# qrp73/SDRPP

Hardware: AMD Instinct MI355X
Metric: IQ Msamples/s through FFT+FIR+demod chain; % HBM roofline at 1/2/4/8 GPU (higher is better)
Workload: dtype f32

## Files before the change

sdrpp_amd/csrc/fft.hip:

```cpp
#include <cmath>
#include <cstring>
#include <cstdlib>
#include <algorithm>
#include <utility>
#include "sdrgpu_internal.h"
#include "fft_stages.h"
#include "fir_rows.h"
#include "fir_tail.h"

#ifndef SDRGPU_PB_NT
#define SDRGPU_PB_NT 1
#endif
#ifndef SDRGPU_PA_CP
#define SDRGPU_PA_CP 2
#endif
namespace sdrgpu {

__device__ __forceinline__ float db_of(float2 X) {
    const float p = X.x * X.x + X.y * X.y;
    int e;
    const float m = frexpf(p, &e);
    const double l = (double)e + (double)__builtin_amdgcn_logf(m);
    return (float)(3.0102999566398119521 * l);
}
// ... 631 lines not shown

namespace op1 {
constexpr int M = 16384;
constexpr int RS = 560;
constexpr int TW512 = 32 * RS;
constexpr int W128 = TW512 + 512;
constexpr int W128D = (W128 + 64) * 8;
constexpr int LDS_BYTES = W128D + 64 * 16;
constexpr int TAB = 512 + 128;
constexpr int TAB64 = 2048 + 128;
}

__device__ __forceinline__ float2 wmul(float2 x, float w) {
#pragma clang fp contract(off)
    return make_float2(x.x * w, x.y * w);
}

__device__ __forceinline__ void dft32(float2* v) {
    constexpr float C[16] = {1.0f, 0.98078528040323044913f, 0.92387953251128675613f, 0.83146961230254523708f,
                             0.70710678118654752440f, 0.55557023301960222474f, 0.38268343236508977173f,
                             0.19509032201612826785f, 0.0f, -0.19509032201612826785f, -0.38268343236508977173f,
                             -0.55557023301960222474f, -0.70710678118654752440f, -0.83146961230254523708f,
                             -0.92387953251128675613f, -0.98078528040323044913f};
    float2 e[16], o[16];
#pragma unroll
    for (int i = 0; i < 16; i++) {
        e[i] = v[2 * i];
        o[i] = v[2 * i + 1];
    }
    dft16(e);
    dft16(o);
#pragma unroll
    for (int k = 0; k < 16; k++) {
        float2 t = o[k];
        if (k == 8) t = mul_negi(t);
        else if (k) t = cmul(t, make_float2(C[k], -C[(k + 8) & 15] * (k < 8 ? -1.0f : 1.0f)));
        v[k] = cadd(e[k], t);
        v[k + 16] = csub(e[k], t);
    }
}

constexpr int k1pSlots = 5;
constexpr int k1pPB = 2;
#ifndef SDRGPU_1P_ABL
#define SDRGPU_1P_ABL 0
#endif
#ifndef SDRGPU_1P_EARLYDMA
#define SDRGPU_1P_EARLYDMA 1
#endif
#ifndef SDRGPU_1P_EARLYW128
#define SDRGPU_1P_EARLYW128 1
#endif
#ifdef SDRGPU_1P_TIMING
__device__ unsigned long long g_1p_t[16384 * 8];
#define T1P(k)                                                                                    \
    do {                                                                                          \
        if (threadIdx.x == 0 && blockIdx.x < 16384) g_1p_t[blockIdx.x * 8 + (k)] = clock64();     \
    } while (0)
#else
#define T1P(k) do {} while (0)
#endif
__device__ __forceinline__ void vfo_half_block(const VfoWork& v, int g, int p) {
    const int lane = threadIdx.x & 63, wave = threadIdx.x >> 6;
#pragma unroll 1
    for (int k = 0; k < 2; k++) {
        const long long seg = (long long)(v.frame0 + g) * 64 + p * 32 + k * 16 + wave * 2 + (lane >> 5);
        fir_rows_segment<32, 5, true, false, 32, 32, true>(v.a, seg, lane);
    }
}
template <bool ZM, bool VFO, bool PAD>
__global__ __launch_bounds__(512) __attribute__((amdgpu_waves_per_eu(1))) void fft_1p_kernel(
    const float2* __restrict__ in, long long frameStride, int frames, const float* __restrict__ win, int nz,
    const float2* __restrict__ tab, const double2* __restrict__ tab64, float* __restrict__ out, float* __restrict__ zpart,
    VfoWork v) {
    using op1::M;
    using op1::RS;
    using op1::TW512;
    using op1::W128;
    extern __shared__ __attribute__((aligned(16))) float2 lds[];
    if constexpr (VFO) {
        if (v.hist && blockIdx.x == gridDim.x - 1) {
            (void)fir_hist_block<float2, true, false>(v.a);
            return;
        }
    }
    const int b = blockIdx.x, k = b >> 3;
    const int f = 8 * (k >> 1) + (b & 7), p = k & 1, r0 = 2 * p;
    if (f >= frames) return;
    T1P(0);
    constexpr bool kDma = !PAD && !(SDRGPU_1P_ABL & 1);
    constexpr bool kVfo = VFO && !(SDRGPU_1P_ABL & 4);
    if constexpr (kVfo && !(kDma && SDRGPU_1P_EARLYDMA)) vfo_half_block(v, f, p);
    T1P(1);
    auto tid = [] {
        int u = threadIdx.x;
        asm volatile("" : "+v"(u));
        return u;
    };
    {
        const int t = threadIdx.x;
        lds[TW512 + t] = tab[t];
        if (t < 64) reinterpret_cast<double2*>(reinterpret_cast<char*>(lds) + op1::W128D)[t] = tab64[2048 + 32 * (r0 + (t >> 5)) + (t & 31)];
    }
    const float fxa = p ? -1.0f : 1.0f, fyb = p ? 1.0f : -1.0f;
    auto combine2 = [&](const float2 (&u)[4], float2& ya, float2& yb) {
        const float2 aa = cadd(u[0], u[2]), qa = cadd(u[1], u[3]), ab = csub(u[0], u[2]), qb = csub(u[1], u[3]);
        ya = make_float2(fmaf(fxa, qa.x, aa.x), fmaf(fxa, qa.y, aa.y));
        yb = make_float2(fmaf(-fyb, qb.y, ab.x), fmaf(fyb, qb.x, ab.y));
    };
    const unsigned lim = PAD ? (unsigned)nz : 65536u;
    const __amdgpu_buffer_rsrc_t rw = brsrc(win, lim * 4u);
    const __amdgpu_buffer_rsrc_t rx = brsrc(in + (long long)f * frameStride, lim * 8u);
    constexpr int PB = k1pPB, NB = 32 / PB;
    float2 za[32], zb[32];
    float2 xv[2][PB][4];
    float wv[2][PB][4];
    auto issue = [&](auto bbc) {
        constexpr int bb = decltype(bbc)::value;
        const int t = tid();
#pragma unroll
        for (int ii = 0; ii < PB; ii++)
#pragma unroll
            for (int j = 0; j < 4; j++) {
                const int n0 = 512 * (PB * bb + ii) + M * j;
                if constexpr (PAD) {
                    xv[bb & 1][ii][j] = __builtin_bit_cast(float2, __builtin_amdgcn_raw_buffer_load_b64(rx, (t + n0) * 8, 0, 0));
                    wv[bb & 1][ii][j] = __builtin_bit_cast(float, __builtin_amdgcn_raw_buffer_load_b32(rw, (t + n0) * 4, 0, 0));
                } else {
                    xv[bb & 1][ii][j] = __builtin_bit_cast(float2, __builtin_amdgcn_raw_buffer_load_b64(rx, t * 8, n0 * 8, 0));
                    wv[bb & 1][ii][j] = __builtin_bit_cast(float, __builtin_amdgcn_raw_buffer_load_b32(rw, t * 4, n0 * 4, 0));
                }
            }
    };
    auto step = [&](auto bbc) {
        constexpr int bb = decltype(bbc)::value;
#pragma unroll
        for (int ii = 0; ii < PB; ii++) {
            float2 u[4];
#pragma unroll
            for (int j = 0; j < 4; j++) u[j] = wmul(xv[bb & 1][ii][j], wv[bb & 1][ii][j]);
            combine2(u, za[PB * bb + ii], zb[PB * bb + ii]);

        }
        if constexpr (bb + 2 < NB) issue(std::integral_constant<int, bb + 2>{});
        __builtin_amdgcn_sched_barrier(0);
    };
    if constexpr (SDRGPU_1P_ABL & 1) {
#pragma unroll
        for (int i = 0; i < 32; i++) {
            za[i] = make_float2((float)(tid() + i), (float)i);
            zb[i] = make_float2((float)i, (float)(tid() - i));
        }
    } else if constexpr (PAD) {
        issue(std::integral_constant<int, 0>{});
        issue(std::integral_constant<int, 1>{});
        static_for<0, NB>(step);
    } else {
        constexpr int S = k1pSlots, SLOT = 24576;
        typedef __attribute__((address_space(3))) char lchar;
        const unsigned ldsBase = (unsigned)(size_t)(lchar*)lds;
        const int wave = __builtin_amdgcn_readfirstlane(threadIdx.x >> 6);
        const char* gb[3];
        unsigned rstep[3], loff[3];
        const float2* xf = in + (long long)f * frameStride;
#pragma unroll
        for (int e = 0; e < 3; e++) {
            const int m = 3 * wave + e;
            const int jx = m >> 2, cx = m & 3, jw = (m - 16) >> 1, cw = (m - 16) & 1;
            gb[e] = m < 16 ? reinterpret_cast<const char*>(xf + M * jx + 128 * cx)
                           : reinterpret_cast<const char*>(win + M * jw + 256 * cw);
            rstep[e] = m < 16 ? 512u * 8u : 512u * 4u;
            loff[e] = m < 16 ? (unsigned)(4096 * jx + 1024 * cx) : (unsigned)(16384 + 2048 * jw + 1024 * cw);
        }
        auto dma = [&](auto ic) {
            constexpr int i = decltype(ic)::value;
            const unsigned lane16 = (unsigned)(tid() & 63) * 16u;
#pragma unroll
            for (int e = 0; e < 3; e++) {
                const char* src = gb[e] + lane16;
                gb[e] += rstep[e];
                asm volatile("" : "+s"(gb[e]));
                const unsigned dst = __builtin_amdgcn_readfirstlane(ldsBase + (unsigned)((i % S) * SLOT) + loff[e]);
                unsigned keep;
                asm volatile("s_mov_b32 %0, m0\n\ts_mov_b32 m0, %2\n\ts_nop 0\n\tglobal_load_lds_dwordx4 %1, off\n\ts_mov_b32 m0, %0"
                             : "=&s"(keep) : "v"(src), "s"(dst) : "memory");
            }
        };
        static_for<0, S - 1>(dma);
        if constexpr (kVfo && SDRGPU_1P_EARLYDMA) vfo_half_block(v, f, p);
        static_for<0, 32>([&](auto ic) {
            constexpr int i = decltype(ic)::value;
            constexpr int younger = (S - 2 < 31 - i) ? S - 2 : 31 - i;
            asm volatile("s_waitcnt vmcnt(%0)" ::"n"(3 * younger) : "memory");
            __builtin_amdgcn_s_barrier();
            asm volatile("" ::: "memory");
            if constexpr (i + S - 1 < 32) dma(std::integral_constant<int, i + S - 1>{});
            const int t = tid();
            const char* slot = reinterpret_cast<const char*>(lds) + (i % S) * SLOT;
            float2 u[4];
#pragma unroll
            for (int j = 0; j < 4; j++) {
                const float2 xx = *reinterpret_cast<const float2*>(slot + 4096 * j + 8 * t);
                const float ww = *reinterpret_cast<const float*>(slot + 16384 + 2048 * j + 4 * t);
                u[j] = wmul(xx, ww);
            }
            combine2(u, za[i], zb[i]);
            __builtin_amdgcn_sched_barrier(0);
        });
    }
    T1P(2);
    float* zf = ZM ? zpart + ((long long)f << 12) : nullptr;
    const __amdgpu_buffer_rsrc_t ro = brsrc(out + ((long long)f << 16), 65536u * 4u);
    float dA[2][16];
    constexpr bool kEarlyW = SDRGPU_1P_EARLYW128 && VFO;
    auto w128mul = [&](float2 (&z)[32], int hh) {
        const double2* w128 = reinterpret_cast<const double2*>(reinterpret_cast<const char*>(lds) + op1::W128D) + 32 * hh;
#pragma unroll
        for (int i = 1; i < 32; i++) {
            const double2 q = zmul(make_double2(z[i].x, z[i].y), w128[i]);
            z[i] = make_float2((float)q.x, (float)q.y);
        }
    };
    auto transform = [&](auto hc, float2 (&z)[32]) {
        constexpr int h = decltype(hc)::value;
        const int r = r0 + h;
        __syncthreads();
        {
            const int t = tid();
            if constexpr (!(kEarlyW && h == 1)) w128mul(z, h);
            dft32(z);
            const double2 st = tab64[4 * t];
            double2 ce = tab64[t * r], co = zmul(ce, st);
            const double2 st2 = zmul(st, st);
            float2* row = lds + pad16(t);
            if constexpr (SDRGPU_1P_ABL & 8) {
                const float2 cf = make_float2((float)ce.x, (float)ce.y), sf = make_float2((float)st.x, (float)st.y);
#pragma unroll
                for (int k2 = 0; k2 < 32; k2++) row[k2 * RS] = cmul(z[k2], k2 & 1 ? sf : cf);
            } else
#pragma unroll
            for (int k2 = 0; k2 < 32; k2 += 2) {
                row[k2 * RS] = cmul(z[k2], make_float2((float)ce.x, (float)ce.y));
                row[(k2 + 1) * RS] = cmul(z[k2 + 1], make_float2((float)co.x, (float)co.y));
                if (k2 < 30) {
                    ce = zmul(ce, st2);
                    co = zmul(co, st2);
                }
            }
        }
        __syncthreads();
        if constexpr (h == 0) T1P(5);
        {
            const int t = tid();
            const int k2 = t >> 4, t0 = t & 15;
            float2 a[32];
            const float2* src = lds + k2 * RS + t0;
#pragma unroll
            for (int t1 = 0; t1 < 32; t1++) a[t1] = src[17 * t1];
            dft32(a);
#pragma unroll
            for (int q1 = 1; q1 < 32; q1++) a[q1] = cmul(a[q1], lds[TW512 + 16 * q1 + t0]);
            __syncthreads();
            float2* dst = lds + k2 * RS + (t0 ^ ((k2 >> 1) & 15));
#pragma unroll
            for (int q1 = 0; q1 < 32; q1++) dst[17 * q1] = a[q1];
        }
        __syncthreads();
        T1P(6 + h);
        static_for<0, 2>([&](auto ec) {
            constexpr int e = decltype(ec)::value;
            const int t = tid();
            const int pe = t + 512 * e, k2 = pe & 31, q1 = pe >> 5, sw = (k2 >> 1) & 15;
            float2 c3[16];
            const float2* src = lds + k2 * RS + 17 * q1;
#pragma unroll
            for (int t0 = 0; t0 < 16; t0++) c3[t0] = src[t0 ^ sw];
            if constexpr (kEarlyW && h == 0 && e == 0) w128mul(zb, 1);
            dft16(c3);
            if constexpr (SDRGPU_1P_ABL & 16) {
                if constexpr (h == 1) {
                    float acc = 0.0f;
#pragma unroll
                    for (int q2 = 0; q2 < 16; q2++) acc += c3[q2].x + c3[q2].y;
                    out[(f << 16) + pe] = acc;
                }
            } else if constexpr (h == 0) {
#pragma unroll
                for (int q2 = 0; q2 < 16; q2++) dA[e][q2] = db_of(c3[q2]);
            } else {
                float dv[16];
                const unsigned vo = (unsigned)(4 * (k2 + 32 * q1) + r0) * 4u;
#pragma unroll
                for (int q2 = 0; q2 < 16; q2++) {
                    dv[q2] = db_of(c3[q2]);
                    __builtin_amdgcn_raw_buffer_store_b64(__builtin_bit_cast(bu2, make_float2(dA[e][q2], dv[q2])), ro, vo,
                                                          q2 * 4096 * 4, 0);
                }
                if constexpr (ZM) {
#pragma unroll
                    for (int q2 = 0; q2 < 16; q2++) dv[q2] = fmaxf(dA[e][q2], dv[q2]);
                    const int lane = t & 63;
                    tr_step<1, 8>(dv, lane);
                    tr_step<2, 4>(dv, lane);
                    tr_step<4, 2>(dv, lane);
                    const int q2 = ((lane & 1) << 3) | ((lane & 2) << 1) | (lane & 4) >> 1;
                    float* zp = zf + ((long long)p << 11) + (k2 >> 3) + 4 * q1 + 128 * q2;
                    zp[0] = dv[0];
                    zp[128] = dv[1];
                }
            }
        });
    };
    if constexpr (SDRGPU_1P_ABL & 2) {
        float2 acc = make_float2(0.0f, 0.0f);
#pragma unroll
        for (int i = 0; i < 32; i++) acc = cadd(acc, cadd(za[i], zb[i]));
        out[(f << 16) + tid()] = acc.x + acc.y;
        return;
    }
    transform(std::integral_constant<int, 0>{}, za);
    T1P(3);
    transform(std::integral_constant<int, 1>{}, zb);
    T1P(4);
}

#ifdef SDRGPU_1P_TIMING
extern "C" int sdrgpu_debug_1p_times(unsigned long long* host, int n) {
    return hipMemcpyFromSymbol(host, HIP_SYMBOL(g_1p_t), sizeof(unsigned long long) * (size_t)n) == hipSuccess ? 0 : -1;
}
#endif

static_assert(TAIL_NT_BIG == 256, "zoom_fold_block's indexing and the fold's block count assume 256 threads");
__device__ __forceinline__ void zoom_fold_block(const float* __restrict__ zpart, int frames, float* __restrict__ zoom, int blk) {
    const long long i = ((long long)blk * 256 + threadIdx.x) * 4;
    if (i >= (long long)frames * 2048) return;
    const long long f = i >> 11, o = i & 2047;
    const float4 a = *reinterpret_cast<const float4*>(zpart + (f << 12) + o);
    const float4 b = *reinterpret_cast<const float4*>(zpart + (f << 12) + 2048 + o);
    const float4 m = make_float4(fmaxf(a.x, b.x), fmaxf(a.y, b.y), fmaxf(a.z, b.z), fmaxf(a.w, b.w));
    if (((uintptr_t)zoom & 15) == 0) {
        *reinterpret_cast<float4*>(zoom + i) = m;
    } else {
        zoom[i] = m.x; zoom[i + 1] = m.y; zoom[i + 2] = m.z; zoom[i + 3] = m.w;
    }
}
__global__ __launch_bounds__(256) void fft_1p_zoom_kernel(const float* __restrict__ zpart, int frames, float* __restrict__ zoom) {
    zoom_fold_block(zpart, frames, zoom, blockIdx.x);
}
__global__ __launch_bounds__(TAIL_NT_BIG) void fft_1p_tail_fold_kernel(TailArgs t, const float* __restrict__ zpart, int frames,
                                                                         float* __restrict__ zoom) {
    extern __shared__ __attribute__((aligned(16))) float2 XS[];
    __shared__ TailGeom gs[TAIL_MAXS];
    const int w = blockIdx.x;
    if (w < t.G) fir_tail_block<TAIL_K_BIG, TAIL_NT_BIG>(t, w, w == t.G - 1, XS, gs);
    else zoom_fold_block(zpart, frames, zoom, w - t.G);
}

struct VfoCall {
    FirArgs a;
    int blocks;
};
__global__ __launch_bounds__(512) __attribute__((amdgpu_waves_per_eu(4))) void fft_passA_vfo_kernel(
    const float2* __restrict__ in, long long frameStride, int frames, const float* __restrict__ win, int nz, int N2,
    int logN, const float2* __restrict__ tw, const float2* __restrict__ tfull, float2* __restrict__ scratch,
    const float2* __restrict__ headp, int nh, SideCopy side, VfoCall v) {
    extern __shared__ __attribute__((aligned(16))) float2 lds[];
    const int ntiles = (N2 / 32) * frames;
    int b = blockIdx.x;
    if (b < ntiles) {
        passA_tile<256, 32>(lds, b, in, frameStride, frames, win, nz, N2, logN, tw, tfull, scratch, headp, nh);
        return;
    }
    b -= ntiles;
    if (b < v.blocks) {
        const int lane = threadIdx.x & 63, wave = threadIdx.x >> 6;
        fir_rows_segment<32, 5, true, false, 32, 32, true>(v.a, ((long long)b * 8 + wave) * 2 + (lane >> 5), lane);
        return;
    }
    b -= v.blocks;
    if (b == 0) {
        fir_hist_copy<float2, true, false>(v.a);
        return;
    }
    const int w = b - 1, nw = gridDim.x - ntiles - v.blocks - 1;
    for (int k = 0; k < side.count; k++)
        for (int i = w * blockDim.x + threadIdx.x; i < side.n[k]; i += nw * blockDim.x) side.dst[k][i] = side.src[k][i];
}

__global__ __launch_bounds__(512) __attribute__((amdgpu_waves_per_eu(4))) void fft_passB_tail_kernel(
    const float2* __restrict__ scratch, int frames, int N1, int logN, const float2* __restrict__ tw, float* __restrict__ out,
    TailArgs t) {
    extern __shared__ __attribute__((aligned(16))) float2 lds[];
    __shared__ TailGeom gs[TAIL_MAXS];
    const int ntiles = (N1 / 32) * frames;
    if ((int)blockIdx.x < ntiles) {
        passB_tile<256, 32, false>(lds, blockIdx.x, scratch, frames, N1, logN, tw, out, nullptr);
        return;
    }
    const int w = blockIdx.x - ntiles;
    fir_tail_block<TAIL_K, TAIL_NT>(t, w, w == t.G - 1, lds, gs);
}

struct FftPlan {
    int device = 0, N = 0, logN = 0, nz = 0;
    int N1 = 0, N2 = 0;
    DevBuf win, tw1, tw2, tfull, scratch, scratch2;
    int chunkFrames = 1;
    int sa = 16, sb = 32;
    float2* cur = nullptr;
    int sa2 = 0;
    int gridA = 0, gridB = 0;
    DevBuf wt;
    hipStream_t own = nullptr;
    PinnedBuf pin_in, pin_out;
    DevBuf dev_in, dev_out;
    int merge = 1;
    StreamOrder order;
    sdrgpu_zoom* zoom = nullptr;
    int zoomSize = 0;
    Fft64Plan* f64 = nullptr;
    static constexpr int kTimed = 256;
    bool timing = false;
    hipEvent_t tev[kTimed][2] = {};
    long long tcalls = 0;
    int vfoFuse = 1;
    int onepass = 0;
    DevBuf tab1p, tab1p64, zpart;
    hipStream_t tailStream = nullptr;
    DevBuf s1T[2], zpartT[2];
    hipEvent_t gdone[2] = {}, tdone[2] = {};
    bool tdoneRec[2] = {};
    long long tcallsT = 0;
};
static int time_mark(FftPlan& p, int which, hipStream_t s) {
    if (!p.timing) return SDRGPU_OK;
    SDRGPU_HIP(hipEventRecord(p.tev[p.tcalls % FftPlan::kTimed][which], s));
    if (which == 1) p.tcalls++;
    return SDRGPU_OK;
}

static int make_twiddles(DevBuf& b, int L, int count = -1, int step = 1) {
    if (count < 0) count = L;
    std::vector<float2> t(count);
    for (int m = 0; m < count; m++) {
        double a = -2.0 * M_PI * (double)((long long)m * step % L) / (double)L;
        t[m] = make_float2((float)std::cos(a), (float)std::sin(a));
    }
    SDRGPU_CHECK(b.ensure(sizeof(float2) * count));
    SDRGPU_HIP(hipMemcpy(b.p, t.data(), sizeof(float2) * count, hipMemcpyHostToDevice));
    return SDRGPU_OK;
}

template <typename K>
static int set_lds(K kernel, size_t bytes) {
    SDRGPU_HIP(hipFuncSetAttribute((const void*)kernel, hipFuncAttributeMaxDynamicSharedMemorySize, (int)bytes));
    return SDRGPU_OK;
}

template <int L, int S>
static int launch_single(const FftPlan& p, const float2* in, long long stride, int frames, float* out, hipStream_t s) {
    auto k = fft_single_kernel<L, S>;
    size_t lds = sizeof(float2) * S * Lds<L>::LS;
    SDRGPU_CHECK(set_lds(k, lds));
    dim3 grid((frames + S - 1) / S);
    hipLaunchKernelGGL(k, grid, dim3(S * L / 16), lds, s, in, stride, frames, p.win.as<float>(), p.nz,
                       p.tw1.as<float2>(), out);
    SDRGPU_HIP(hipGetLastError());
    return SDRGPU_OK;
}

template <int L, int S>
static int launch_passA(const FftPlan& p, const float2* in, long long stride, int frames, hipStream_t s,
                        const float2* headp = nullptr, int nh = 0, const SideCopy* side = nullptr) {
    auto k = fft_passA_kernel<L, S>;
    size_t lds = sizeof(float2) * (S * Lds<L>::LS + (L == 256 ? L + 256 : 0));
    SDRGPU_CHECK(set_lds(k, lds));
    SideCopy sc{};
    int spare = 0;
    if (side && side->count > 0) {
// ... 135 lines not shown
    set_error("fft: unsupported N2 %d", p.N2);
    return SDRGPU_EARG;
}

}

using namespace sdrgpu;

struct sdrgpu_fft {
    FftPlan p;
};

static int fft_upload_window(sdrgpu_fft* h, const float* window, int nz) {
    if (nz <= 0 || nz > h->p.N) { set_error("fft: nz %d out of range (N %d)", nz, h->p.N); return SDRGPU_EARG; }
    SDRGPU_SET_DEVICE(h->p.device);
    SDRGPU_CHECK(h->p.win.ensure(sizeof(float) * nz));
    SDRGPU_HIP(hipMemcpy(h->p.win.p, window, sizeof(float) * nz, hipMemcpyHostToDevice));
    h->p.nz = nz;
    return SDRGPU_OK;
}

extern "C" int sdrgpu_fft_create(sdrgpu_fft** out, int device, int fftSize, int nz, int windowType) {
    if (!out) { set_error("fft_create: null handle"); return SDRGPU_EARG; }
    *out = nullptr;
    int logN = 0;
    while ((1 << logN) < fftSize) logN++;
    if (fftSize < 64 || fftSize > (1 << 20) || (1 << logN) != fftSize) {
        set_error("fft_create: size %d must be a power of two in [64, 2^20]", fftSize);
        return SDRGPU_EARG;
    }
    SDRGPU_SET_DEVICE(device);
    sdrgpu_fft* h = new sdrgpu_fft();
    FftPlan& p = h->p;
    p.device = device; p.N = fftSize; p.logN = logN;
    int rc;
    if (fftSize <= 4096) {
        p.N1 = p.N2 = 0;
        rc = make_twiddles(p.tw1, fftSize);
    } else {
        p.N1 = 1 << ((logN + 1) / 2);
        p.N2 = fftSize / p.N1;
        rc = make_twiddles(p.tw1, p.N1);
        if (rc >= 0) rc = make_twiddles(p.tw2, p.N2);

        long long chunkMB = 128;
        if (p.N1 == 1024 && p.N2 == 1024) chunkMB = 64;
        if (const char* e = tuning_env("SDRGPU_FFT_CHUNK_MB")) chunkMB = std::max(1, atoi(e));
        if (p.N1 == 256 && p.N2 == 256) p.sa = p.sb = 32;
        if (const char* e = tuning_env("SDRGPU_FFT_MERGE")) p.merge = atoi(e);
        p.chunkFrames = std::max(1, (int)((chunkMB << 20) / ((long long)fftSize * 8)));
        p.sa2 = p.N1 >= 512 ? 16 : 0;
        p.onepass = fftSize == 65536 ? 2 : 0;
        if (const char* e = tuning_env("SDRGPU_FFT_1P")) p.onepass = atoi(e);
        if (rc >= 0 && fftSize == 65536) {
            std::vector<float2> t(op1::TAB);
            auto w = [&](long long m) {
                const double a = -2.0 * M_PI * (double)(m % fftSize) / (double)fftSize;
                return make_float2((float)std::cos(a), (float)std::sin(a));
            };
            for (int q1 = 0; q1 < 32; q1++)
                for (int t0 = 0; t0 < 16; t0++) t[16 * q1 + t0] = w(128LL * t0 * q1);
            for (int r = 0; r < 4; r++)
                for (int i = 0; i < 32; i++) t[512 + 32 * r + i] = w(512LL * r * i);
            std::vector<double2> t64(op1::TAB64);
            auto w64 = [&](long long m) {
                const double a = -2.0 * M_PI * (double)(m % fftSize) / (double)fftSize;
                return make_double2(std::cos(a), std::sin(a));
            };
            for (int m = 0; m < 2048; m++) t64[m] = w64(m);
            for (int r = 0; r < 4; r++)
                for (int i = 0; i < 32; i++) t64[2048 + 32 * r + i] = w64(512LL * r * i);
            rc = p.tab1p.ensure(sizeof(float2) * t.size());
            if (rc >= 0) rc = p.tab1p64.ensure(sizeof(double2) * t64.size());
            if (rc >= 0 && (hipMemcpy(p.tab1p.p, t.data(), sizeof(float2) * t.size(), hipMemcpyHostToDevice) != hipSuccess ||
                            hipMemcpy(p.tab1p64.p, t64.data(), sizeof(double2) * t64.size(), hipMemcpyHostToDevice) != hipSuccess)) {
                set_error("fft: twiddle upload failed");
                rc = SDRGPU_EHIP;
            }
        }
        if (rc >= 0 && p.N1 == 1024 && p.N2 == 1024) {
            std::vector<double2> t(512);
            for (int j = 0; j < 256; j++) {
                const double a = -2.0 * M_PI * (double)(256 * j) / (double)fftSize;
                const double b = -2.0 * M_PI * (double)j / (double)fftSize;
                t[j] = make_double2(std::cos(a), std::sin(a));
                t[256 + j] = make_double2(std::cos(b), std::sin(b));
            }
            rc = p.wt.ensure(sizeof(double2) * t.size());
            if (rc >= 0 && hipMemcpy(p.wt.p, t.data(), sizeof(double2) * t.size(), hipMemcpyHostToDevice) != hipSuccess) {
                set_error("fft: twiddle upload failed");
                rc = SDRGPU_EHIP;
            }
        }
        if (rc >= 0) {
            std::vector<float2> t((size_t)fftSize);
            for (int k1 = 0; k1 < p.N1; k1++)
                for (int n2 = 0; n2 < p.N2; n2++) {
                    const long long m = ((long long)n2 * k1) % fftSize;
                    const double a = -2.0 * M_PI * (double)m / (double)fftSize;
                    t[(size_t)k1 * p.N2 + n2] = make_float2((float)std::cos(a), (float)std::sin(a));
                }
            rc = p.tfull.ensure(sizeof(float2) * t.size());
            if (rc >= 0 && hipMemcpy(p.tfull.p, t.data(), sizeof(float2) * t.size(), hipMemcpyHostToDevice) != hipSuccess) {
                set_error("fft: twiddle upload failed");
                rc = SDRGPU_EHIP;
            }
        }
    }
    if (rc >= 0 && hipStreamCreateWithFlags(&p.own, hipStreamNonBlocking) != hipSuccess) {
        set_error("fft_create: hipStreamCreate failed");
        rc = SDRGPU_EHIP;
    }
    if (rc >= 0) rc = sdrgpu_fft_set_window_type(h, windowType, nz);
    if (rc < 0) { sdrgpu_fft_destroy(h); return rc; }
    *out = h;
    return SDRGPU_OK;
}

extern "C" int sdrgpu_fft_set_window(sdrgpu_fft* h, const float* window, int nz) {
    if (!h || !window) { set_error("fft_set_window: null argument"); return SDRGPU_EARG; }
    return fft_upload_window(h, window, nz);
}

extern "C" int sdrgpu_fft_set_window_type(sdrgpu_fft* h, int windowType, int nz) {
    if (!h) { set_error("fft_set_window_type: null handle"); return SDRGPU_EARG; }
    if (nz <= 0 || nz > h->p.N) { set_error("fft: nz %d out of range (N %d)", nz, h->p.N); return SDRGPU_EARG; }
    std::vector<float> w(nz);
    SDRGPU_CHECK(create_window(windowType, w.data(), nz, 1));
    return fft_upload_window(h, w.data(), nz);
}

extern "C" int sdrgpu_fft_size(sdrgpu_fft* h) { return h ? h->p.N : SDRGPU_EARG; }

extern "C" int sdrgpu_fft_set_precision(sdrgpu_fft* h, int mode) {
    if (!h || mode < 0 || mode > 1) { set_error("fft_set_precision: bad argument"); return SDRGPU_EARG; }
    FftPlan& p = h->p;
    SDRGPU_SET_DEVICE(p.device);
    SDRGPU_HIP(hipDeviceSynchronize());
    if (mode == 0 && p.f64) {
        fft64_destroy(p.f64);
        p.f64 = nullptr;
    } else if (mode == 1 && !p.f64) {
        SDRGPU_CHECK(fft64_create(&p.f64, p.N));
    }
    return SDRGPU_OK;
}
extern "C" int sdrgpu_fft_get_precision(sdrgpu_fft* h) { return h ? (h->p.f64 ? 1 : 0) : SDRGPU_EARG; }

static bool zoom_fusable(const FftPlan& p, int zoomSize) {
    return p.N1 == 256 && p.N2 == 256 && p.sa == 32 && p.sb == 32 && zoomSize * 32 == p.N;
}

template <bool ZM, bool VFO>
static int launch_1p(FftPlan& p, const float2* in, long long stride, int frames, float* out, float* zoom, VfoWork v,
                     hipStream_t s, bool fold = true, DevBuf* zpb = nullptr) {
    const bool pad = p.nz < 65536 || (stride & 1) || ((uintptr_t)in & 15);
    DevBuf& zp = zpb ? *zpb : p.zpart;
    if (ZM) SDRGPU_CHECK(zp.ensure(sizeof(float) * 2 * 2048 * (size_t)frames));
    const int g = 16 * ((frames + 7) / 8) + (VFO && v.hist ? 1 : 0);
    auto k = pad ? fft_1p_kernel<ZM, VFO, true> : fft_1p_kernel<ZM, VFO, false>;
    SDRGPU_CHECK(set_lds(k, op1::LDS_BYTES));
    hipLaunchKernelGGL(k, dim3(g), dim3(512), op1::LDS_BYTES, s, in, stride, frames, p.win.as<float>(), p.nz,
                       p.tab1p.as<float2>(), p.tab1p64.as<double2>(), out, ZM ? zp.as<float>() : nullptr, v);
    SDRGPU_HIP(hipGetLastError());
    if (ZM && fold) {
        const long long n = (long long)frames * 2048 / 4;
        hipLaunchKernelGGL(fft_1p_zoom_kernel, dim3((unsigned)((n + 255) / 256)), dim3(256), 0, s, zp.as<float>(),
                           frames, zoom);
        SDRGPU_HIP(hipGetLastError());
    }
    return SDRGPU_OK;
}
constexpr int k1pMinFrames = 64;
static bool onepass_ok(const FftPlan& p, int frames) {
    return p.N == 65536 && p.tab1p.p && !p.f64 && (p.onepass == 1 || (p.onepass == 2 && frames >= k1pMinFrames));
}

static int fft_execute_body(sdrgpu_fft* h, const void* in, long long frameStride, int frames, float* out, float* zoom,
                            hipStream_t s);
static int fft_execute(sdrgpu_fft* h, const void* in, long long frameStride, int frames, float* out, float* zoom,
                       hipStream_t s) {
    SDRGPU_CHECK(time_mark(h->p, 0, s));
    const int rc = fft_execute_body(h, in, frameStride, frames, out, zoom, s);
    if (rc < 0) return rc;
    SDRGPU_CHECK(time_mark(h->p, 1, s));
    return rc;
}
static int fft_execute_body(sdrgpu_fft* h, const void* in, long long frameStride, int frames, float* out, float* zoom,
                            hipStream_t s) {
    FftPlan& p = h->p;
    const float2* x = (const float2*)in;
    if (p.f64) return fft64_execute(p.f64, x, frameStride, frames, p.win.as<float>(), p.nz, out, s);
    if (p.N1 == 0) {
        SDRGPU_CHECK(dispatch_single(p, x, frameStride, frames, out, s));
        return frames;
    }
    if (onepass_ok(p, frames)) {
        const int rc = zoom ? launch_1p<true, false>(p, x, frameStride, frames, out, zoom, VfoWork{}, s)
                            : launch_1p<false, false>(p, x, frameStride, frames, out, nullptr, VfoWork{}, s);
        if (rc < 0) return rc;
        return frames;
    }
    const long long zw = p.N / 32;
    auto zoomAt = [&](long long f0) { return zoom ? zoom + f0 * zw : nullptr; };
    const bool paired = p.sa2 > 0 && (frameStride % 2) == 0 && ((uintptr_t)in & 15) == 0;
    const int nchunks = (frames + p.chunkFrames - 1) / p.chunkFrames;
    SDRGPU_CHECK(p.scratch.ensure((size_t)std::min(p.chunkFrames, frames) * p.N * sizeof(float2)));
    if (p.merge && nchunks > 1 && merged_supported(p, paired)) {
        SDRGPU_CHECK(p.scratch2.ensure(p.scratch.bytes));
        float2* sc[2] = {p.scratch.as<float2>(), p.scratch2.as<float2>()};
        p.cur = sc[0];
        SDRGPU_CHECK(dispatch_passA(p, x, frameStride, std::min(p.chunkFrames, frames), s));
        for (int c = 1; c < nchunks; c++) {
            const int fB = (c - 1) * p.chunkFrames, nfB = p.chunkFrames;
            const int fA = c * p.chunkFrames, nfA = std::min(p.chunkFrames, frames - fA);
            const float2* xa = x + (long long)fA * frameStride;
// ... 394 lines not shown
```

Measured before the change: 179,400.

## Make one-pass FFT kernel persistent with cross-item DMA prefetch

Converts the one-pass 65536-point FFT kernel into a persistent grid sized to resident occupancy (CUs times blocks per CU) that loops over frame/half work items. While finishing the transform of one item, it issues the LDS DMA prologue for the next item so input loads overlap the tail compute. This is meant to remove per-block launch and prologue overhead and hide load latency at item boundaries. In exchange it adds extra barriers and waitcnts, kernarg reloads per iteration, and register pressure. The padded path still processes one item per block.

```diff
diff --git a/sdrpp_amd/csrc/fft.hip b/sdrpp_amd/csrc/fft.hip
--- a/sdrpp_amd/csrc/fft.hip
+++ b/sdrpp_amd/csrc/fft.hip
@@ -707,46 +707,65 @@
 #define SDRGPU_1P_EARLYW128 1
 #endif
 #ifdef SDRGPU_1P_TIMING
-__device__ unsigned long long g_1p_t[16384 * 8];
-#define T1P(k)                                                                                    \
-    do {                                                                                          \
-        if (threadIdx.x == 0 && blockIdx.x < 16384) g_1p_t[blockIdx.x * 8 + (k)] = clock64();     \
+constexpr int k1pStamps = 10;
+__device__ unsigned long long g_1p_t[16384 * k1pStamps];
+#define T1P_AT(item, k)                                                                               \
+    do {                                                                                              \
+        if (threadIdx.x == 0 && (item) < 16384) g_1p_t[(item) * k1pStamps + (k)] = clock64();         \
+    } while (0)
+#define T1P_CU(item)                                                                                  \
+    do {                                                                                              \
+        if (threadIdx.x == 0 && (item) < 16384) {                                                     \
+            unsigned hw, xcc;                                                                         \
+            asm volatile("s_getreg_b32 %0, hwreg(HW_REG_HW_ID)\n\ts_getreg_b32 %1, hwreg(HW_REG_XCC_ID)" \
+                         : "=s"(hw), "=s"(xcc));                                                      \
+            g_1p_t[(item) * k1pStamps + 8] = (unsigned long long)xcc << 32 | hw;                       \
+        }                                                                                             \
     } while (0)
 #else
-#define T1P(k) do {} while (0)
+#define T1P_AT(item, k) do {} while (0)
+#define T1P_CU(item) do {} while (0)
 #endif
+#define T1P(k) T1P_AT(b, k)
 __device__ __forceinline__ void vfo_half_block(const VfoWork& v, int g, int p) {
-    const int lane = threadIdx.x & 63, wave = threadIdx.x >> 6;
+    int u = threadIdx.x;
+    asm volatile("" : "+v"(u));
+    const int lane = u & 63, wave = u >> 6;
 #pragma unroll 1
     for (int k = 0; k < 2; k++) {
         const long long seg = (long long)(v.frame0 + g) * 64 + p * 32 + k * 16 + wave * 2 + (lane >> 5);
         fir_rows_segment<32, 5, true, false, 32, 32, true>(v.a, seg, lane);
     }
 }
+struct Args1p {
+    const float2* in;
+    long long frameStride;
+    int frames;
+    const float* win;
+    int nz;
+    const float2* tab;
+    const double2* tab64;
+    float* out;
+    float* zpart;
+    VfoWork v;
+};
 template <bool ZM, bool VFO, bool PAD>
-__global__ __launch_bounds__(512) __attribute__((amdgpu_waves_per_eu(1))) void fft_1p_kernel(
-    const float2* __restrict__ in, long long frameStride, int frames, const float* __restrict__ win, int nz,
-    const float2* __restrict__ tab, const double2* __restrict__ tab64, float* __restrict__ out, float* __restrict__ zpart,
-    VfoWork v) {
+__global__ __launch_bounds__(512) __attribute__((amdgpu_waves_per_eu(1))) void fft_1p_kernel(Args1p ka) {
     using op1::M;
     using op1::RS;
     using op1::TW512;
     using op1::W128;
     extern __shared__ __attribute__((aligned(16))) float2 lds[];
     if constexpr (VFO) {
-        if (v.hist && blockIdx.x == gridDim.x - 1) {
-            (void)fir_hist_block<float2, true, false>(v.a);
+        if (ka.v.hist && blockIdx.x == gridDim.x - 1) {
+            (void)fir_hist_block<float2, true, false>(ka.v.a);
             return;
         }
     }
-    const int b = blockIdx.x, k = b >> 3;
-    const int f = 8 * (k >> 1) + (b & 7), p = k & 1, r0 = 2 * p;
-    if (f >= frames) return;
-    T1P(0);
+    const int frames = ka.frames, G = (int)gridDim.x - (VFO && ka.v.hist ? 1 : 0), items = 16 * ((frames + 7) >> 3);
+    int p = (blockIdx.x >> 3) & 1;
     constexpr bool kDma = !PAD && !(SDRGPU_1P_ABL & 1);
     constexpr bool kVfo = VFO && !(SDRGPU_1P_ABL & 4);
-    if constexpr (kVfo && !(kDma && SDRGPU_1P_EARLYDMA)) vfo_half_block(v, f, p);
-    T1P(1);
     auto tid = [] {
         int u = threadIdx.x;
         asm volatile("" : "+v"(u));
@@ -754,229 +773,284 @@
     };
     {
         const int t = threadIdx.x;
-        lds[TW512 + t] = tab[t];
-        if (t < 64) reinterpret_cast<double2*>(reinterpret_cast<char*>(lds) + op1::W128D)[t] = tab64[2048 + 32 * (r0 + (t >> 5)) + (t & 31)];
-    }
-    const float fxa = p ? -1.0f : 1.0f, fyb = p ? 1.0f : -1.0f;
-    auto combine2 = [&](const float2 (&u)[4], float2& ya, float2& yb) {
-        const float2 aa = cadd(u[0], u[2]), qa = cadd(u[1], u[3]), ab = csub(u[0], u[2]), qb = csub(u[1], u[3]);
-        ya = make_float2(fmaf(fxa, qa.x, aa.x), fmaf(fxa, qa.y, aa.y));
-        yb = make_float2(fmaf(-fyb, qb.y, ab.x), fmaf(fyb, qb.x, ab.y));
+        lds[TW512 + t] = ka.tab[t];
+        if (t < 64) reinterpret_cast<double2*>(reinterpret_cast<char*>(lds) + op1::W128D)[t] = ka.tab64[2048 + 32 * (2 * p + (t >> 5)) + (t & 31)];
+    }
+    const unsigned lim = PAD ? (unsigned)ka.nz : 65536u;
+    const __amdgpu_buffer_rsrc_t rw = brsrc(ka.win, lim * 4u);
+    constexpr int S = k1pSlots, SLOT = 24576;
+    typedef __attribute__((address_space(3))) char lchar;
+    lchar* const lds3 = (lchar*)lds;
+    unsigned ldsBase = (unsigned)(size_t)lds3;
+    int wave = __builtin_amdgcn_readfirstlane(threadIdx.x >> 6);
+    const char* gb[3];
+    unsigned goff[3], rstep[3], loff[3];
+#pragma unroll
+    for (int e = 0; e < 3; e++) {
+        const int m = 3 * wave + e;
+        const int jx = m >> 2, cx = m & 3, jw = (m - 16) >> 1, cw = (m - 16) & 1;
+        goff[e] = m < 16 ? (unsigned)(M * jx + 128 * cx) * 8u : (unsigned)(M * jw + 256 * cw) * 4u;
+        rstep[e] = m < 16 ? 512u * 8u : 512u * 4u;
+        loff[e] = m < 16 ? (unsigned)(4096 * jx + 1024 * cx) : (unsigned)(16384 + 2048 * jw + 1024 * cw);
+    }
+    auto set_rows = [&](const float2* xf, const float* w) {
+#pragma unroll
+        for (int e = 0; e < 3; e++)
+            gb[e] = (3 * wave + e < 16 ? reinterpret_cast<const char*>(xf) : reinterpret_cast<const char*>(w)) + goff[e];
     };
-    const unsigned lim = PAD ? (unsigned)nz : 65536u;
-    const __amdgpu_buffer_rsrc_t rw = brsrc(win, lim * 4u);
-    const __amdgpu_buffer_rsrc_t rx = brsrc(in + (long long)f * frameStride, lim * 8u);
-    constexpr int PB = k1pPB, NB = 32 / PB;
-    float2 za[32], zb[32];
-    float2 xv[2][PB][4];
-    float wv[2][PB][4];
-    auto issue = [&](auto bbc) {
-        constexpr int bb = decltype(bbc)::value;
-        const int t = tid();
-#pragma unroll
-        for (int ii = 0; ii < PB; ii++)
-#pragma unroll
-            for (int j = 0; j < 4; j++) {
-                const int n0 = 512 * (PB * bb + ii) + M * j;
-                if constexpr (PAD) {
-                    xv[bb & 1][ii][j] = __builtin_bit_cast(float2, __builtin_amdgcn_raw_buffer_load_b64(rx, (t + n0) * 8, 0, 0));
-                    wv[bb & 1][ii][j] = __builtin_bit_cast(float, __builtin_amdgcn_raw_buffer_load_b32(rw, (t + n0) * 4, 0, 0));
-                } else {
-                    xv[bb & 1][ii][j] = __builtin_bit_cast(float2, __builtin_amdgcn_raw_buffer_load_b64(rx, t * 8, n0 * 8, 0));
-                    wv[bb & 1][ii][j] = __builtin_bit_cast(float, __builtin_amdgcn_raw_buffer_load_b32(rw, t * 4, n0 * 4, 0));
+    auto dma = [&](auto ic) {
+        constexpr int i = decltype(ic)::value;
+        const unsigned lane16 = (unsigned)(tid() & 63) * 16u;
+#pragma unroll
+        for (int e = 0; e < 3; e++) {
+            const char* src = gb[e] + lane16;
+            gb[e] += rstep[e];
+            asm volatile("" : "+s"(gb[e]));
+            const unsigned dst = __builtin_amdgcn_readfirstlane(ldsBase + (unsigned)((i % S) * SLOT) + loff[e]);
+            unsigned keep;
+            asm volatile("s_mov_b32 %0, m0\n\ts_mov_b32 m0, %2\n\ts_nop 0\n\tglobal_load_lds_dwordx4 %1, off\n\ts_mov_b32 m0, %0"
+                         : "=&s"(keep) : "v"(src), "s"(dst) : "memory");
+        }
+    };
+    bool pre = false;
+#pragma unroll 1
+    for (int b = blockIdx.x; b < items; b += G) {
+        asm volatile("" : "+s"(b), "+s"(p));
+        if constexpr (kDma) {
+            asm volatile("" : "+s"(ldsBase), "+s"(wave));
+#pragma unroll
+            for (int e = 0; e < 3; e++) asm volatile("" : "+s"(goff[e]), "+s"(rstep[e]), "+s"(loff[e]));
+        }
+        typedef const __attribute__((address_space(4))) char kchar;
+        kchar* kp = (kchar*)__builtin_amdgcn_kernarg_segment_ptr();
+        asm volatile("" : "+s"(kp));
+        const Args1p& ia = *reinterpret_cast<const Args1p*>((const char*)kp);
+        const float2* __restrict__ in = ia.in;
+        const long long frameStride = ia.frameStride;
+        const float* __restrict__ win = ia.win;
+        const double2* __restrict__ tab64 = ia.tab64;
+        float* __restrict__ out = ia.out;
+        float* __restrict__ zpart = ia.zpart;
+        const VfoWork& v = ia.v;
+        const int f = 8 * (b >> 4) + (b & 7), r0 = 2 * p;
+        lchar* l3 = lds3;
+        asm volatile("" : "+s"(l3));
+        float2* const lds = reinterpret_cast<float2*>((char*)l3);
+        const float fxa = p ? -1.0f : 1.0f, fyb = p ? 1.0f : -1.0f;
+        auto combine2 = [&](const float2 (&u)[4], float2& ya, float2& yb) {
+            const float2 aa = cadd(u[0], u[2]), qa = cadd(u[1], u[3]), ab = csub(u[0], u[2]), qb = csub(u[1], u[3]);
+            ya = make_float2(fmaf(fxa, qa.x, aa.x), fmaf(fxa, qa.y, aa.y));
+            yb = make_float2(fmaf(-fyb, qb.y, ab.x), fmaf(fyb, qb.x, ab.y));
+        };
+        if (f >= frames) {
+            if constexpr (PAD) break;
+            continue;
+        }
+        T1P(0);
+        T1P_CU(b);
+        if constexpr (kVfo && !(kDma && SDRGPU_1P_EARLYDMA)) vfo_half_block(v, f, p);
+        T1P(1);
+        const __amdgpu_buffer_rsrc_t rx = brsrc(in + (long long)f * frameStride, lim * 8u);
+        constexpr int PB = k1pPB, NB = 32 / PB;
+        float2 za[32], zb[32];
+        float2 xv[2][PB][4];
+        float wv[2][PB][4];
+        auto issue = [&](auto bbc) {
+            constexpr int bb = decltype(bbc)::value;
+            const int t = tid();
+#pragma unroll
+            for (int ii = 0; ii < PB; ii++)
+#pragma unroll
+                for (int j = 0; j < 4; j++) {
+                    const int n0 = 512 * (PB * bb + ii) + M * j;
+                    if constexpr (PAD) {
+                        xv[bb & 1][ii][j] = __builtin_bit_cast(float2, __builtin_amdgcn_raw_buffer_load_b64(rx, (t + n0) * 8, 0, 0));
+                        wv[bb & 1][ii][j] = __builtin_bit_cast(float, __builtin_amdgcn_raw_buffer_load_b32(rw, (t + n0) * 4, 0, 0));
+                    } else {
+                        xv[bb & 1][ii][j] = __builtin_bit_cast(float2, __builtin_amdgcn_raw_buffer_load_b64(rx, t * 8, n0 * 8, 0));
+                        wv[bb & 1][ii][j] = __builtin_bit_cast(float, __builtin_amdgcn_raw_buffer_load_b32(rw, t * 4, n0 * 4, 0));
+                    }
+                }
+        };
+        auto step = [&](auto bbc) {
+            constexpr int bb = decltype(bbc)::value;
+#pragma unroll
+            for (int ii = 0; ii < PB; ii++) {
+                float2 u[4];
+#pragma unroll
+                for (int j = 0; j < 4; j++) u[j] = wmul(xv[bb & 1][ii][j], wv[bb & 1][ii][j]);
+                combine2(u, za[PB * bb + ii], zb[PB * bb + ii]);
+
+            }
+            if constexpr (bb + 2 < NB) issue(std::integral_constant<int, bb + 2>{});
+            __builtin_amdgcn_sched_barrier(0);
+        };
+        if constexpr (SDRGPU_1P_ABL & 1) {
+#pragma unroll
+            for (int i = 0; i < 32; i++) {
+                za[i] = make_float2((float)(tid() + i), (float)i);
+                zb[i] = make_float2((float)i, (float)(tid() - i));
+            }
+        } else if constexpr (PAD) {
+            issue(std::integral_constant<int, 0>{});
+            issue(std::integral_constant<int, 1>{});
+            static_for<0, NB>(step);
+        } else {
+            if (!pre) {
+                set_rows(in + (long long)f * frameStride, win);
+                static_for<0, S - 1>(dma);
+            }
+            if constexpr (kVfo && SDRGPU_1P_EARLYDMA) vfo_half_block(v, f, p);
+            if (pre) asm volatile("s_waitcnt vmcnt(0)" ::: "memory");
+            static_for<0, 32>([&](auto ic) {
+                constexpr int i = decltype(ic)::value;
+                constexpr int younger = (S - 2 < 31 - i) ? S - 2 : 31 - i;
+                asm volatile("s_waitcnt vmcnt(%0)" ::"n"(3 * younger) : "memory");
+                __builtin_amdgcn_s_barrier();
+                asm volatile("" ::: "memory");
+                if constexpr (i == 0) T1P(9);
+                if constexpr (i + S - 1 < 32) dma(std::integral_constant<int, i + S - 1>{});
+                const int t = tid();
+                const char* slot = reinterpret_cast<const char*>(lds) + (i % S) * SLOT;
+                float2 u[4];
+#pragma unroll
+                for (int j = 0; j < 4; j++) {
+                    const float2 xx = *reinterpret_cast<const float2*>(slot + 4096 * j + 8 * t);
+                    const float ww = *reinterpret_cast<const float*>(slot + 16384 + 2048 * j + 4 * t);
+                    u[j] = wmul(xx, ww);
+                }
+                combine2(u, za[i], zb[i]);
+                __builtin_amdgcn_sched_barrier(0);
+            });
+        }
+        T1P(2);
+        float* zf = ZM ? zpart + ((long long)f << 12) : nullptr;
+        const __amdgpu_buffer_rsrc_t ro = brsrc(out + ((long long)f << 16), 65536u * 4u);
+        float dA[2][16];
+        constexpr bool kEarlyW = SDRGPU_1P_EARLYW128 && VFO;
+        auto w128mul = [&](float2 (&z)[32], int hh) {
+            const double2* w128 = reinterpret_cast<const double2*>(reinterpret_cast<const char*>(lds) + op1::W128D) + 32 * hh;
+#pragma unroll
+            for (int i = 1; i < 32; i++) {
+                const double2 q = zmul(make_double2(z[i].x, z[i].y), w128[i]);
+                z[i] = make_float2((float)q.x, (float)q.y);
+            }
+        };
+        auto prefetch = [&] {
+            int bn = b + G;
+            asm volatile("" : "+s"(bn));
+            const int fn = 8 * (bn >> 4) + (bn & 7);
+            pre = bn < items && fn < frames;
+            if (pre) {
+                asm volatile("s_waitcnt lgkmcnt(0)\n\ts_barrier" ::: "memory");
+                set_rows(in + (long long)fn * frameStride, win);
+                static_for<0, S - 1>(dma);
+            }
+        };
+        auto transform = [&](auto hc, float2 (&z)[32]) {
+            constexpr int h = decltype(hc)::value;
+            const int r = r0 + h;
+            __syncthreads();
+            {
+                const int t = tid();
+                if constexpr (!(kEarlyW && h == 1)) w128mul(z, h);
+                dft32(z);
+                const double2 st = tab64[4 * t];
+                double2 ce = tab64[t * r], co = zmul(ce, st);
+                const double2 st2 = zmul(st, st);
+                float2* row = lds + pad16(t);
+                if constexpr (SDRGPU_1P_ABL & 8) {
+                    const float2 cf = make_float2((float)ce.x, (float)ce.y), sf = make_float2((float)st.x, (float)st.y);
+#pragma unroll
+                    for (int k2 = 0; k2 < 32; k2++) row[k2 * RS] = cmul(z[k2], k2 & 1 ? sf : cf);
+                } else
+#pragma unroll
+                for (int k2 = 0; k2 < 32; k2 += 2) {
+                    row[k2 * RS] = cmul(z[k2], make_float2((float)ce.x, (float)ce.y));
+                    row[(k2 + 1) * RS] = cmul(z[k2 + 1], make_float2((float)co.x, (float)co.y));
+                    if (k2 < 30) {
+                        ce = zmul(ce, st2);
+                        co = zmul(co, st2);
+                    }
                 }
             }
-    };
-    auto step = [&](auto bbc) {
-        constexpr int bb = decltype(bbc)::value;
-#pragma unroll
-        for (int ii = 0; ii < PB; ii++) {
-            float2 u[4];
-#pragma unroll
-            for (int j = 0; j < 4; j++) u[j] = wmul(xv[bb & 1][ii][j], wv[bb & 1][ii][j]);
-            combine2(u, za[PB * bb + ii], zb[PB * bb + ii]);
-
-        }
-        if constexpr (bb + 2 < NB) issue(std::integral_constant<int, bb + 2>{});
-        __builtin_amdgcn_sched_barrier(0);
-    };
-    if constexpr (SDRGPU_1P_ABL & 1) {
-#pragma unroll
-        for (int i = 0; i < 32; i++) {
-            za[i] = make_float2((float)(tid() + i), (float)i);
-            zb[i] = make_float2((float)i, (float)(tid() - i));
-        }
-    } else if constexpr (PAD) {
-        issue(std::integral_constant<int, 0>{});
-        issue(std::integral_constant<int, 1>{});
-        static_for<0, NB>(step);
-    } else {
-        constexpr int S = k1pSlots, SLOT = 24576;
-        typedef __attribute__((address_space(3))) char lchar;
-        const unsigned ldsBase = (unsigned)(size_t)(lchar*)lds;
-        const int wave = __builtin_amdgcn_readfirstlane(threadIdx.x >> 6);
-        const char* gb[3];
-        unsigned rstep[3], loff[3];
-        const float2* xf = in + (long long)f * frameStride;
-#pragma unroll
-        for (int e = 0; e < 3; e++) {
-            const int m = 3 * wave + e;
-            const int jx = m >> 2, cx = m & 3, jw = (m - 16) >> 1, cw = (m - 16) & 1;
-            gb[e] = m < 16 ? reinterpret_cast<const char*>(xf + M * jx + 128 * cx)
-                           : reinterpret_cast<const char*>(win + M * jw + 256 * cw);
-            rstep[e] = m < 16 ? 512u * 8u : 512u * 4u;
-            loff[e] = m < 16 ? (unsigned)(4096 * jx + 1024 * cx) : (unsigned)(16384 + 2048 * jw + 1024 * cw);
-        }
-        auto dma = [&](auto ic) {
-            constexpr int i = decltype(ic)::value;
-            const unsigned lane16 = (unsigned)(tid() & 63) * 16u;
-#pragma unroll
-            for (int e = 0; e < 3; e++) {
-                const char* src = gb[e] + lane16;
-                gb[e] += rstep[e];
-                asm volatile("" : "+s"(gb[e]));
-                const unsigned dst = __builtin_amdgcn_readfirstlane(ldsBase + (unsigned)((i % S) * SLOT) + loff[e]);
-                unsigned keep;
-                asm volatile("s_mov_b32 %0, m0\n\ts_mov_b32 m0, %2\n\ts_nop 0\n\tglobal_load_lds_dwordx4 %1, off\n\ts_mov_b32 m0, %0"
-                             : "=&s"(keep) : "v"(src), "s"(dst) : "memory");
+            __syncthreads();
+            if constexpr (h == 0) T1P(5);
+            {
+                const int t = tid();
+                const int k2 = t >> 4, t0 = t & 15;
+                float2 a[32];
+                const float2* src = lds + k2 * RS + t0;
+#pragma unroll
+                for (int t1 = 0; t1 < 32; t1++) a[t1] = src[17 * t1];
+                dft32(a);
+#pragma unroll
+                for (int q1 = 1; q1 < 32; q1++) a[q1] = cmul(a[q1], lds[TW512 + 16 * q1 + t0]);
+                __syncthreads();
+                float2* dst = lds + k2 * RS + (t0 ^ ((k2 >> 1) & 15));
+#pragma unroll
+                for (int q1 = 0; q1 < 32; q1++) dst[17 * q1] = a[q1];
             }
+            __syncthreads();
+            T1P(6 + h);
+            static_for<0, 2>([&](auto ec) {
+                constexpr int e = decltype(ec)::value;
+                const int t = tid();
+                const int pe = t + 512 * e, k2 = pe & 31, q1 = pe >> 5, sw = (k2 >> 1) & 15;
+                float2 c3[16];
+                const float2* src = lds + k2 * RS + 17 * q1;
+#pragma unroll
+                for (int t0 = 0; t0 < 16; t0++) c3[t0] = src[t0 ^ sw];
+                if constexpr (kEarlyW && h == 0 && e == 0) w128mul(zb, 1);
+                if constexpr (kDma && h == 1 && e == 1) prefetch();
+                dft16(c3);
+                if constexpr (SDRGPU_1P_ABL & 16) {
+                    if constexpr (h == 1) {
+                        float acc = 0.0f;
+#pragma unroll
+                        for (int q2 = 0; q2 < 16; q2++) acc += c3[q2].x + c3[q2].y;
+                        out[(f << 16) + pe] = acc;
+                    }
+                } else if constexpr (h == 0) {
+#pragma unroll
+                    for (int q2 = 0; q2 < 16; q2++) dA[e][q2] = db_of(c3[q2]);
+                } else {
+                    float dv[16];
+                    const unsigned vo = (unsigned)(4 * (k2 + 32 * q1) + r0) * 4u;
+#pragma unroll
+                    for (int q2 = 0; q2 < 16; q2++) {
+                        dv[q2] = db_of(c3[q2]);
+                        __builtin_amdgcn_raw_buffer_store_b64(__builtin_bit_cast(bu2, make_float2(dA[e][q2], dv[q2])), ro, vo,
+                                                              q2 * 4096 * 4, 0);
+                    }
+                    if constexpr (ZM) {
+#pragma unroll
+                        for (int q2 = 0; q2 < 16; q2++) dv[q2] = fmaxf(dA[e][q2], dv[q2]);
+                        const int lane = t & 63;
+                        tr_step<1, 8>(dv, lane);
+                        tr_step<2, 4>(dv, lane);
+                        tr_step<4, 2>(dv, lane);
+                        const int q2 = ((lane & 1) << 3) | ((lane & 2) << 1) | (lane & 4) >> 1;
+                        float* zp = zf + ((long long)p << 11) + (k2 >> 3) + 4 * q1 + 128 * q2;
+                        zp[0] = dv[0];
+                        zp[128] = dv[1];
+                    }
+                }
+            });
         };
-        static_for<0, S - 1>(dma);
-        if constexpr (kVfo && SDRGPU_1P_EARLYDMA) vfo_half_block(v, f, p);
-        static_for<0, 32>([&](auto ic) {
-            constexpr int i = decltype(ic)::value;
-            constexpr int younger = (S - 2 < 31 - i) ? S - 2 : 31 - i;
-            asm volatile("s_waitcnt vmcnt(%0)" ::"n"(3 * younger) : "memory");
-            __builtin_amdgcn_s_barrier();
-            asm volatile("" ::: "memory");
-            if constexpr (i + S - 1 < 32) dma(std::integral_constant<int, i + S - 1>{});
-            const int t = tid();
-            const char* slot = reinterpret_cast<const char*>(lds) + (i % S) * SLOT;
-            float2 u[4];
-#pragma unroll
-            for (int j = 0; j < 4; j++) {
-                const float2 xx = *reinterpret_cast<const float2*>(slot + 4096 * j + 8 * t);
-                const float ww = *reinterpret_cast<const float*>(slot + 16384 + 2048 * j + 4 * t);
-                u[j] = wmul(xx, ww);
-            }
-            combine2(u, za[i], zb[i]);
-            __builtin_amdgcn_sched_barrier(0);
-        });
-    }
-    T1P(2);
-    float* zf = ZM ? zpart + ((long long)f << 12) : nullptr;
-    const __amdgpu_buffer_rsrc_t ro = brsrc(out + ((long long)f << 16), 65536u * 4u);
-    float dA[2][16];
-    constexpr bool kEarlyW = SDRGPU_1P_EARLYW128 && VFO;
-    auto w128mul = [&](float2 (&z)[32], int hh) {
-        const double2* w128 = reinterpret_cast<const double2*>(reinterpret_cast<const char*>(lds) + op1::W128D) + 32 * hh;
-#pragma unroll
-        for (int i = 1; i < 32; i++) {
-            const double2 q = zmul(make_double2(z[i].x, z[i].y), w128[i]);
-            z[i] = make_float2((float)q.x, (float)q.y);
-        }
-    };
-    auto transform = [&](auto hc, float2 (&z)[32]) {
-        constexpr int h = decltype(hc)::value;
-        const int r = r0 + h;
-        __syncthreads();
-        {
-            const int t = tid();
-            if constexpr (!(kEarlyW && h == 1)) w128mul(z, h);
-            dft32(z);
-            const double2 st = tab64[4 * t];
-            double2 ce = tab64[t * r], co = zmul(ce, st);
-            const double2 st2 = zmul(st, st);
-            float2* row = lds + pad16(t);
-            if constexpr (SDRGPU_1P_ABL & 8) {
-                const float2 cf = make_float2((float)ce.x, (float)ce.y), sf = make_float2((float)st.x, (float)st.y);
-#pragma unroll
-                for (int k2 = 0; k2 < 32; k2++) row[k2 * RS] = cmul(z[k2], k2 & 1 ? sf : cf);
-            } else
-#pragma unroll
-            for (int k2 = 0; k2 < 32; k2 += 2) {
-                row[k2 * RS] = cmul(z[k2], make_float2((float)ce.x, (float)ce.y));
-                row[(k2 + 1) * RS] = cmul(z[k2 + 1], make_float2((float)co.x, (float)co.y));
-                if (k2 < 30) {
-                    ce = zmul(ce, st2);
-                    co = zmul(co, st2);
-                }
-            }
-        }
-        __syncthreads();
-        if constexpr (h == 0) T1P(5);
-        {
-            const int t = tid();
-            const int k2 = t >> 4, t0 = t & 15;
-            float2 a[32];
-            const float2* src = lds + k2 * RS + t0;
-#pragma unroll
-            for (int t1 = 0; t1 < 32; t1++) a[t1] = src[17 * t1];
-            dft32(a);
-#pragma unroll
-            for (int q1 = 1; q1 < 32; q1++) a[q1] = cmul(a[q1], lds[TW512 + 16 * q1 + t0]);
-            __syncthreads();
-            float2* dst = lds + k2 * RS + (t0 ^ ((k2 >> 1) & 15));
-#pragma unroll
-            for (int q1 = 0; q1 < 32; q1++) dst[17 * q1] = a[q1];
-        }
-        __syncthreads();
-        T1P(6 + h);
-        static_for<0, 2>([&](auto ec) {
-            constexpr int e = decltype(ec)::value;
-            const int t = tid();
-            const int pe = t + 512 * e, k2 = pe & 31, q1 = pe >> 5, sw = (k2 >> 1) & 15;
-            float2 c3[16];
-            const float2* src = lds + k2 * RS + 17 * q1;
-#pragma unroll
-            for (int t0 = 0; t0 < 16; t0++) c3[t0] = src[t0 ^ sw];
-            if constexpr (kEarlyW && h == 0 && e == 0) w128mul(zb, 1);
-            dft16(c3);
-            if constexpr (SDRGPU_1P_ABL & 16) {
-                if constexpr (h == 1) {
-                    float acc = 0.0f;
-#pragma unroll
-                    for (int q2 = 0; q2 < 16; q2++) acc += c3[q2].x + c3[q2].y;
-                    out[(f << 16) + pe] = acc;
-                }
-            } else if constexpr (h == 0) {
-#pragma unroll
-                for (int q2 = 0; q2 < 16; q2++) dA[e][q2] = db_of(c3[q2]);
-            } else {
-                float dv[16];
-                const unsigned vo = (unsigned)(4 * (k2 + 32 * q1) + r0) * 4u;
-#pragma unroll
-                for (int q2 = 0; q2 < 16; q2++) {
-                    dv[q2] = db_of(c3[q2]);
-                    __builtin_amdgcn_raw_buffer_store_b64(__builtin_bit_cast(bu2, make_float2(dA[e][q2], dv[q2])), ro, vo,
-                                                          q2 * 4096 * 4, 0);
-                }
-                if constexpr (ZM) {
-#pragma unroll
-                    for (int q2 = 0; q2 < 16; q2++) dv[q2] = fmaxf(dA[e][q2], dv[q2]);
-                    const int lane = t & 63;
-                    tr_step<1, 8>(dv, lane);
-                    tr_step<2, 4>(dv, lane);
-                    tr_step<4, 2>(dv, lane);
-                    const int q2 = ((lane & 1) << 3) | ((lane & 2) << 1) | (lane & 4) >> 1;
-                    float* zp = zf + ((long long)p << 11) + (k2 >> 3) + 4 * q1 + 128 * q2;
-                    zp[0] = dv[0];
-                    zp[128] = dv[1];
-                }
-            }
-        });
-    };
-    if constexpr (SDRGPU_1P_ABL & 2) {
-        float2 acc = make_float2(0.0f, 0.0f);
-#pragma unroll
-        for (int i = 0; i < 32; i++) acc = cadd(acc, cadd(za[i], zb[i]));
-        out[(f << 16) + tid()] = acc.x + acc.y;
-        return;
-    }
-    transform(std::integral_constant<int, 0>{}, za);
-    T1P(3);
-    transform(std::integral_constant<int, 1>{}, zb);
-    T1P(4);
+        if constexpr (SDRGPU_1P_ABL & 2) {
+            float2 acc = make_float2(0.0f, 0.0f);
+#pragma unroll
+            for (int i = 0; i < 32; i++) acc = cadd(acc, cadd(za[i], zb[i]));
+            out[(f << 16) + tid()] = acc.x + acc.y;
+            continue;
+        }
+        transform(std::integral_constant<int, 0>{}, za);
+        T1P(3);
+        transform(std::integral_constant<int, 1>{}, zb);
+        T1P(4);
+        if constexpr (PAD) break;
+    }
 }
 
 #ifdef SDRGPU_1P_TIMING
@@ -1080,6 +1154,8 @@
     long long tcalls = 0;
     int vfoFuse = 1;
     int onepass = 0;
+    int grid1p = -1;
+    int res1p[4] = {};
     DevBuf tab1p, tab1p64, zpart;
     hipStream_t tailStream = nullptr;
     DevBuf s1T[2], zpartT[2];
@@ -1321,6 +1397,7 @@
         p.sa2 = p.N1 >= 512 ? 16 : 0;
         p.onepass = fftSize == 65536 ? 2 : 0;
         if (const char* e = tuning_env("SDRGPU_FFT_1P")) p.onepass = atoi(e);
+        if (const char* e = tuning_env("SDRGPU_FFT_1P_GRID")) p.grid1p = std::max(0, atoi(e));
         if (rc >= 0 && fftSize == 65536) {
             std::vector<float2> t(op1::TAB);
             auto w = [&](long long m) {
@@ -1426,11 +1503,28 @@
     const bool pad = p.nz < 65536 || (stride & 1) || ((uintptr_t)in & 15);
     DevBuf& zp = zpb ? *zpb : p.zpart;
     if (ZM) SDRGPU_CHECK(zp.ensure(sizeof(float) * 2 * 2048 * (size_t)frames));
-    const int g = 16 * ((frames + 7) / 8) + (VFO && v.hist ? 1 : 0);
     auto k = pad ? fft_1p_kernel<ZM, VFO, true> : fft_1p_kernel<ZM, VFO, false>;
     SDRGPU_CHECK(set_lds(k, op1::LDS_BYTES));
-    hipLaunchKernelGGL(k, dim3(g), dim3(512), op1::LDS_BYTES, s, in, stride, frames, p.win.as<float>(), p.nz,
-                       p.tab1p.as<float2>(), p.tab1p64.as<double2>(), out, ZM ? zp.as<float>() : nullptr, v);
+    const int items = 16 * ((frames + 7) / 8);
+    int G = items;
+    if (p.grid1p != 0 && !pad) {
+        int n = p.grid1p;
+        if (n < 0) {
+            int& res = p.res1p[2 * ZM + VFO];
+            if (!res) {
+                int per = 0, cus = 0;
+                SDRGPU_HIP(hipOccupancyMaxActiveBlocksPerMultiprocessor(&per, (const void*)k, 512, op1::LDS_BYTES));
+                SDRGPU_HIP(hipDeviceGetAttribute(&cus, hipDeviceAttributeMultiprocessorCount, p.device));
+                res = std::max(1, per) * std::max(1, cus);
+            }
+            n = res;
+        }
+        G = std::min(items, std::max(16, n / 16 * 16));
+    }
+    const int g = G + (VFO && v.hist ? 1 : 0);
+    hipLaunchKernelGGL(k, dim3(g), dim3(512), op1::LDS_BYTES, s,
+                       Args1p{in, stride, frames, p.win.as<float>(), p.nz, p.tab1p.as<float2>(), p.tab1p64.as<double2>(), out,
+                              ZM ? zp.as<float>() : nullptr, v});
     SDRGPU_HIP(hipGetLastError());
     if (ZM && fold) {
         const long long n = (long long)frames * 2048 / 4;
```

After: 186,200 (median of 6 runs). 1.04x the previous value.
